# Excalibur-SLE/spmv

Hardware: AMD Instinct MI355X
Metric: fp64 CG iters/sec (SpMV effective GB/s vs HBM roofline) (higher is better)
Workload: dtype f64

## Files before the change

spmv_amd/csrc/hip/common.h:

```cpp
#pragma once

#include <mutex>
#include <vector>

#include <hip/hip_runtime.h>

#include <cstdint>
#include <cstdlib>

#include "spmv_hip.h"

struct spmv_hip_ctx {
  int device = 0;
  int num_cus = 0;
  hipStream_t stream = nullptr;
  int dot_blocks = 0;
  int64_t blas1_nt_min_elems = (int64_t)1 << 24;
  int64_t lx_min_nnz = (int64_t)1 << 20;
  int64_t lx_max_x_bytes = INT64_MAX;
  int lx_dma = 1;
  int lx_codes = 1;
  int lx_narrow_values = 1;
  int release_csr = 0;
  int64_t xw_min_nnz = (int64_t)1 << 20;
  int64_t xw_min_x_bytes = (int64_t)128 << 20;
  int xw_probe = 1;
  int csr_in_place = 0;
  int64_t lat_min_nnz = (int64_t)1 << 20;
  int bake_general = 1;
  int wdia_half = 1;
  int const_diagonals = 1;
  int const_tile = 4;
  int64_t sj_min_nnz = (int64_t)1 << 20;
  int sj_max_chunks = 432;
  int sj_wpb = 0;
  int sj_unit = 0;
  int sj_sigma = 1;
  int sym_sj_long_permille = 50;
  int sym_sj_long_rows = 1;
  int put_timeout_ms = 60000;
  std::vector<const int32_t*> watched;
  std::mutex watched_mutex;
  int poisson_skew_ppm = 0;
  int poisson_stencil = 7;
};
// ... 105 lines not shown
```

spmv_amd/csrc/hip/csr_plan.h:

```cpp
#pragma once

#include "common.h"

#include <chrono>
#include <cstdio>

constexpr int kRows = kBlock;

typedef double f64x2 __attribute__((ext_vector_type(2)));
typedef float f32x4 __attribute__((ext_vector_type(4)));
typedef int i32x2 __attribute__((ext_vector_type(2)));
typedef int i32x4 __attribute__((ext_vector_type(4)));

template <typename T>
struct VecOf;
template <>
struct VecOf<double> {
  static constexpr int V = 2;
  using val_t = f64x2;
  using col_t = i32x2;
};
template <>
struct VecOf<float> {
  static constexpr int V = 4;
// ... 288 lines not shown
  bool structure_baked() const
  {
    return row_list || lx_lidx || lat_tab || slat_mask || t_ptr || lxw_rec
           || xw_rec || wdia_val || sj_lenperm;
  }
  uint16_t* lx_lidx = nullptr;
  int32_t* lx_tab = nullptr;
  int lx = 0;
  int lx_chunks = 2;
  int lx_staged = 0;
  int lx_blocks = 0;
  int32_t* lxw_rec = nullptr;
  int lxw = 0;
  int lxw_max_cnt = 0;
  int lxw_max_pieces = 0;
  int lxw_blocks_per_cu = 0;
  uint8_t* lx_code = nullptr;
  int lx4 = 0;
  int lx4_blocks = 0;
  int lx4_lut = 1;
  float* lx_val32 = nullptr;
  const void* lx32_values0 = nullptr;
  int lx_v32 = 0;
  int32_t* xw_rec = nullptr;
  int xw = 0;
  int xw_staged = 0;
  int xw_max_cnt = 0, xw_max_pieces = 0;
  struct XwProbe* xw_probe = nullptr;
  int32_t* lat_tab = nullptr;
  uint8_t* lat_mask = nullptr;
  int lat = 0;
  int lat_blocks = 0;
  int lat_blocks_per_cu = 4;
  int lat_xcd_group = 0;
  int lat_chain = 1;

  int lattice_d1 = 0, lattice_d2 = 0;

  int32_t* zw_table = nullptr;
  int zw_slots = 0;
  int zw_grid = 0;
  int zw_segments = 0;
  int64_t zw_d2 = 0;
  int zwalk = 0;

  RowBlockOrder row_block_order(int nrb) const
// ... 71 lines not shown
                      const double* diagonal, double alpha, const double* in,
                      double beta, double* out, DotOut dot);
int spmv_slat_run_f32(const spmv_hip_csr_plan* pl, hipStream_t st,
                      const int32_t* rowptr, const float* values,
                      const float* diagonal, float alpha, const float* in,
                      float beta, float* out);
void spmv_sdia_free(spmv_hip_csr_plan* pl);
int spmv_sdia_tile_build(spmv_hip_csr_plan* pl, int R, int segments, bool force);
int spmv_sdia_bake_f64(spmv_hip_csr_plan* pl, const double* values,
                       const double* diagonal, hipStream_t st);
int spmv_sdia_bake_f32(spmv_hip_csr_plan* pl, const float* values,
                       const float* diagonal, hipStream_t st);
int spmv_sdia_grid(const spmv_hip_csr_plan* pl);
int spmv_sdia_bake_f32f64(spmv_hip_csr_plan* pl, const float* values32,
                          hipStream_t st);
int spmv_sdia_run_f32f64(const spmv_hip_csr_plan* pl, hipStream_t st,
                         double alpha, const double* in, double beta,
                         double* out, DotOut dot);
int spmv_sdia_run_f64(const spmv_hip_csr_plan* pl, hipStream_t st, double alpha,
                      const double* in, double beta, double* out, DotOut dot);
int spmv_sdia_run_f32(const spmv_hip_csr_plan* pl, hipStream_t st, float alpha,
                      const float* in, float beta, float* out);
int spmv_lxw_grid(const spmv_hip_csr_plan* pl, int elem_bytes);
int spmv_lxw_run_f64(const spmv_hip_csr_plan* pl, hipStream_t st,
                     const int32_t* rowptr, const int32_t* colind,
                     const double* values, double alpha, const double* in,
                     double beta, double* out, DotOut dot);
int spmv_lxw_run_f32f64(const spmv_hip_csr_plan* pl, hipStream_t st,
                        const int32_t* rowptr, const int32_t* colind,
                        const float* values, double alpha, const double* in,
                        double beta, double* out, DotOut dot);
int spmv_xw_grid(const spmv_hip_csr_plan* pl, int elem_bytes);
int spmv_xw_run_f64(const spmv_hip_csr_plan* pl, hipStream_t st,
                    const int32_t* rowptr, const int32_t* colind,
                    const double* values, double alpha, const double* in,
                    double beta, double* out, DotOut dot);
int spmv_xw_run_f32(const spmv_hip_csr_plan* pl, hipStream_t st,
                    const int32_t* rowptr, const int32_t* colind,
                    const float* values, float alpha, const float* in,
                    float beta, float* out);
int spmv_lxw_run_f32(const spmv_hip_csr_plan* pl, hipStream_t st,
                     const int32_t* rowptr, const int32_t* colind,
                     const float* values, float alpha, const float* in,
                     float beta, float* out);
void spmv_wdia_free(spmv_hip_csr_plan* pl);
int spmv_wdia_walk_build(spmv_hip_csr_plan* pl, int segments, bool force);
// ... 56 lines not shown
```

spmv_amd/csrc/hip/runtime.hip:

```cpp
#include "common.h"

#include <cstdio>
#include <cstring>
#include <new>

bool spmv_ctx_watch(spmv_hip_ctx* ctx, const int32_t* word, bool add)
{
  std::lock_guard<std::mutex> lock(ctx->watched_mutex);
  auto& ws = ctx->watched;
  if (add) {
    try {
      ws.push_back(word);
    } catch (...) {
      return false;
    }
    return true;
  }
  for (size_t i = 0; i < ws.size(); ++i)
    if (ws[i] == word) {
      ws[i] = ws.back();
      ws.pop_back();
      break;
    }
  return true;
// ... 121 lines not shown
}

int spmv_hip_ctx_get_option(const spmv_hip_ctx* ctx, const char* key, int64_t* value)
{
  SPMV_REQUIRE(ctx && key && value);
  if (!strcmp(key, "release_csr"))
    *value = ctx->release_csr;
  else if (!strcmp(key, "put_timeout_ms"))
    *value = ctx->put_timeout_ms;
  else if (!strcmp(key, "xw_min_nnz"))
    *value = ctx->xw_min_nnz;
  else if (!strcmp(key, "xw_min_x_bytes"))
    *value = ctx->xw_min_x_bytes;
  else if (!strcmp(key, "xw_probe"))
    *value = ctx->xw_probe;
  else if (!strcmp(key, "csr_in_place"))
    *value = ctx->csr_in_place;
  else if (!strcmp(key, "lx_min_nnz"))
    *value = ctx->lx_min_nnz;
  else if (!strcmp(key, "lat_min_nnz"))
    *value = ctx->lat_min_nnz;
  else if (!strcmp(key, "lx_narrow_values"))
    *value = ctx->lx_narrow_values;
  else if (!strcmp(key, "sj_min_nnz"))
    *value = ctx->sj_min_nnz;
  else
    return SPMV_HIP_EINVAL;
  return SPMV_HIP_OK;
}

int spmv_hip_ctx_set_option(spmv_hip_ctx* ctx, const char* key, int64_t value)
{
  SPMV_REQUIRE(ctx && key);
  if (!strcmp(key, "blas1_nt_min_elems")) {
    SPMV_REQUIRE(value >= 0);
    ctx->blas1_nt_min_elems = value;
    return SPMV_HIP_OK;
  }
  if (!strcmp(key, "lx_max_x_bytes")) {
    SPMV_REQUIRE(value >= 0);
    ctx->lx_max_x_bytes = value;
    return SPMV_HIP_OK;
  }
  if (!strcmp(key, "lx_min_nnz")) {
    SPMV_REQUIRE(value >= 0);
    ctx->lx_min_nnz = value;
// ... 27 lines not shown
  if (!strcmp(key, "lat_min_nnz")) {
    SPMV_REQUIRE(value >= 0);
    ctx->lat_min_nnz = value;
    return SPMV_HIP_OK;
  }
  if (!strcmp(key, "poisson_skew_ppm")) {
    SPMV_REQUIRE(value >= 0 && value < 1000000);
    ctx->poisson_skew_ppm = (int)value;
    return SPMV_HIP_OK;
  }
  if (!strcmp(key, "lx_dma")) {
    SPMV_REQUIRE(value == 0 || value == 1);
    ctx->lx_dma = (int)value;
    return SPMV_HIP_OK;
  }
  if (!strcmp(key, "lx_codes")) {
    SPMV_REQUIRE(value == 0 || value == 1);
    ctx->lx_codes = (int)value;
    return SPMV_HIP_OK;
  }
  if (!strcmp(key, "lx_narrow_values")) {
    SPMV_REQUIRE(value == 0 || value == 1);
    ctx->lx_narrow_values = (int)value;
    return SPMV_HIP_OK;
  }
  if (!strcmp(key, "poisson_stencil")) {
    SPMV_REQUIRE(value == 7 || value == 27);
    ctx->poisson_stencil = (int)value;
    return SPMV_HIP_OK;
  }
  if (!strcmp(key, "const_diagonals")) {
    SPMV_REQUIRE(value == 0 || value == 1);
    ctx->const_diagonals = (int)value;
    return SPMV_HIP_OK;
  }
  if (!strcmp(key, "const_tile")) {
    SPMV_REQUIRE(value == 1 || value == 2 || value == 4);
    ctx->const_tile = (int)value;
    return SPMV_HIP_OK;
  }
  if (!strcmp(key, "wdia_half")) {
    SPMV_REQUIRE(value == 0 || value == 1);
    ctx->wdia_half = (int)value;
    return SPMV_HIP_OK;
  }
  if (!strcmp(key, "sj_min_nnz")) {
// ... 264 lines not shown
```

spmv_amd/csrc/hip/spmv_csr_plan.hip:

```cpp
#include "csr_plan.h"

#include <hipcub/hipcub.hpp>

#include <algorithm>
#include <chrono>
#include <cstring>
#include <new>
#include <utility>
#include <vector>

#include "plan_malloc.h"

thread_local int64_t spmv_plan_mem_ns = 0;

namespace
{
struct MemClock {
  spmv_hip_csr_plan* pl;
  int64_t t0;
  explicit MemClock(spmv_hip_csr_plan* p = nullptr) : pl(p), t0(spmv_plan_mem_ns) {}
  ~MemClock()
  {
    if (pl)
      pl->plan_mem_us += (int)((spmv_plan_mem_ns - t0) / 1000);
// ... 65 lines not shown
}

extern "C" {

int spmv_hip_csr_plan_create(spmv_hip_ctx* ctx, int32_t num_rows,
                             int32_t num_cols, int64_t num_non_zeros,
                             const int32_t* rowptr, const int32_t* colind,
                             int symmetric, int algo, spmv_hip_csr_plan** plan)
{
  SPMV_REQUIRE(ctx && plan && num_rows >= 0 && num_cols >= 0
               && num_non_zeros >= 0);
  SPMV_REQUIRE(num_non_zeros == 0 || (rowptr && colind));
  if (num_non_zeros > 0) {
    SPMV_SET_DEVICE(ctx);
    SPMV_CHECK_HIP(hipStreamSynchronize(spmv_stream(ctx, nullptr)));
  }
  const auto t_begin = std::chrono::steady_clock::now();
  if (num_non_zeros > INT32_MAX)
    return SPMV_HIP_ERANGE;
  spmv_hip_csr_plan* pl = new (std::nothrow) spmv_hip_csr_plan;
  if (!pl)
    return SPMV_HIP_ENOMEM;
  pl->ctx = ctx;
  MemClock mem_clock(pl);
  pl->num_rows = num_rows;
  pl->num_cols = num_cols;
  pl->nnz = num_non_zeros;
  pl->symmetric = symmetric != 0;
  pl->rowptr0 = rowptr;
  pl->colind0 = colind;
  const double avg = num_rows > 0 ? (double)num_non_zeros / num_rows : 0.0;
  if (algo == SPMV_HIP_ALGO_AUTO) {
    if (!symmetric && num_non_zeros > 0 && num_non_zeros * 4 < num_rows)
      algo = SPMV_HIP_ALGO_ROWLIST;
    else
      algo = (avg <= 64.0 || num_non_zeros >= ctx->sj_min_nnz)
                 ? SPMV_HIP_ALGO_ROWBLOCK
                 : SPMV_HIP_ALGO_VECTOR;
  }
  if (algo < SPMV_HIP_ALGO_ROWBLOCK || algo > SPMV_HIP_ALGO_ROWLIST
      || (algo == SPMV_HIP_ALGO_ROWLIST && (symmetric || num_non_zeros == 0))) {
    mem_clock.pl = nullptr;
    delete pl;
    return SPMV_HIP_EINVAL;
  }
  pl->algo = algo;
// ... 366 lines not shown
    SPMV_REQUIRE(value >= 1 && value <= kBlocksPerCU);
    plan->blocks_per_cu = value;
    if (plan->zw_table && !plan->lat_tab && !plan->symmetric
        && !plan->sdia_val)
      return spmv_zwalk_order_build(plan, plan->zw_d2, spmv_walk_grid(plan), 0,
                                    true);
  } else if (!strcmp(key, "lx")) {
    SPMV_REQUIRE(value == 0 || plan->lx_lidx);
    plan->lx = value != 0;
  } else if (!strcmp(key, "lxw")) {
    SPMV_REQUIRE(value == 0 || plan->lxw_rec);
    plan->lxw = value != 0;
    if (plan->zw_table && plan->lx_lidx && !plan->lat_tab)
      return spmv_zwalk_order_build(plan, plan->zw_d2, spmv_walk_grid(plan), 0,
                                    true);
  } else if (!strcmp(key, "lx4")) {
    SPMV_REQUIRE(value == 0 || value == 1);
    SPMV_REQUIRE(value == 0 || plan->lx_code);
    plan->lx4 = value;
  } else if (!strcmp(key, "lx_v32")) {
    SPMV_REQUIRE(value == 0 || value == 1);
    SPMV_REQUIRE(value == 0 || plan->lx_val32);
    plan->lx_v32 = value;
  } else if (!strcmp(key, "lx4_lut")) {
    SPMV_REQUIRE(value == 1 || value == 2);
    plan->lx4_lut = value;
  } else if (!strcmp(key, "xw")) {
    SPMV_REQUIRE(value == 0 || plan->xw_rec);
    plan->xw = value != 0;
    if (plan->xw_probe && value) {
      plan->xw_probe->decided = 1;
      plan->xw_probe->use_xw = 1;
    }
    if (plan->zw_table && plan->xw_rec && !plan->lat_tab && !plan->lx_lidx)
      return spmv_zwalk_order_build(plan, plan->zw_d2, spmv_walk_grid(plan), 0,
                                    true);
  } else if (!strcmp(key, "xw_probe")) {
    SPMV_REQUIRE((value == 0 || value == 1) && plan->xw_rec);
    if (!plan->xw_probe)
      plan->xw_probe = new (std::nothrow) XwProbe;
    SPMV_REQUIRE(plan->xw_probe);
    xw_probe_drop_events(plan->xw_probe);
    *plan->xw_probe = XwProbe();
    plan->xw_probe->decided = value ? 0 : 1;
  } else if (!strcmp(key, "lxw_blocks_per_cu")) {
    SPMV_REQUIRE(value >= 0 && value <= kBlocksPerCU);
// ... 353 lines not shown
    *value = plan->lattice_d1;
  else if (!strcmp(key, "lattice_d2"))
    *value = plan->lattice_d2;
  else if (!strcmp(key, "lat"))
    *value = plan->lat;
  else if (!strcmp(key, "lat_chain"))
    *value = plan->lat_chain;
  else if (!strcmp(key, "lat_blocks"))
    *value = plan->lat_blocks;
  else if (!strcmp(key, "lx"))
    *value = plan->lx;
  else if (!strcmp(key, "lxw"))
    *value = plan->lxw && plan->lxw_rec ? 1 : 0;
  else if (!strcmp(key, "lx4"))
    *value = plan->lx4 && plan->lx_code ? 1 : 0;
  else if (!strcmp(key, "lx4_blocks"))
    *value = plan->lx_code ? plan->lx4_blocks : 0;
  else if (!strcmp(key, "lx4_all"))
    *value = plan->lx_code && plan->lx4_blocks == plan->lx_staged ? 1 : 0;
  else if (!strcmp(key, "lx4_lut"))
    *value = plan->lx4_lut;
  else if (!strcmp(key, "lx_v32"))
    *value = plan->lx_v32 && plan->lx_val32 ? 1 : 0;
  else if (!strcmp(key, "lxw_grid"))
    *value = plan->lxw_rec ? spmv_lxw_grid(plan, 8) : 0;
  else if (!strcmp(key, "lx_staged"))
    *value = plan->lx_staged;
  else if (!strcmp(key, "lx_blocks"))
    *value = plan->lx_blocks;
  else if (!strcmp(key, "blocks_per_cu"))
    *value = plan->blocks_per_cu;
  else if (!strcmp(key, "nontemporal"))
    *value = plan->nontemporal;
  else
    return spmv_tr_get(plan, key, value);
  return SPMV_HIP_OK;
}

}
```

spmv_amd/csrc/hip/spmv_lxw.hip:

```cpp
#include "csr_plan.h"
#include "lat_dma.h"

#include <new>
#include <type_traits>

namespace
{

struct LxwBlock {
  int rb;
  int nwin;
  int32_t a;
  int32_t cnt;
  int np;
  int own;
  int coded;
};

template <int REC>
__device__ __forceinline__ int32_t lxw_fetch(int rb,
                                             const int32_t* __restrict__ rec)
{
  int32_t w = 0;
  if (rb >= 0) {
// ... 25 lines not shown
  T y0;
};

template <typename T>
__device__ __forceinline__ LxwRegs<T> lxw_loads(const LxwBlock& blk, int t,
                                                int32_t num_rows,
                                                const int32_t* __restrict__ rowptr,
                                                const T* __restrict__ in, T beta,
                                                const T* __restrict__ out)
{
  LxwRegs<T> g;
  g.lo = g.hi = 0;
  g.y0 = T(0);
  if (blk.rb >= 0) {
    const int32_t r = blk.rb * kRows + t;
    if (r < num_rows) {
      g.lo = rowptr[r];
      g.hi = rowptr[r + 1];
      if (beta != T(0))
        g.y0 = out[r];
    }
  }
  return g;
}

template <typename TV, typename T, bool DOT, bool NT, bool TAB, bool XW, int C4>
__global__ __launch_bounds__(kBlock) void csr_lxw_kernel(
    int32_t num_rows, int32_t num_cols, int64_t nnz,
    const int32_t* __restrict__ rowptr, const int32_t* __restrict__ colind,
    const TV* __restrict__ values, const uint16_t* __restrict__ lidx,
    const uint8_t* __restrict__ code, const int32_t* __restrict__ rec, T alpha, const T* __restrict__ in, T beta,
    T* __restrict__ out, DotOut dot, RowBlockOrder ord, int vcap, int lcap,
    int xcap)
{
  using IDX = typename std::conditional<XW, int32_t, uint16_t>::type;
  constexpr int REC = XW ? kXwRec : kLxwRec;
  constexpr int IA = 16 / (int)sizeof(IDX) - 1;
  constexpr int V = 16 / (int)sizeof(TV);
  constexpr int E = 16 / (int)sizeof(T);
  constexpr int PL = kLxwPiece / E;
  extern __shared__ __attribute__((aligned(16))) unsigned char smem[];
  TV* const s_val = reinterpret_cast<TV*>(smem);
  IDX* const s_lidx
      = reinterpret_cast<IDX*>(smem + 2 * (size_t)vcap * sizeof(TV));
  T* const s_x = reinterpret_cast<T*>(smem + 2 * (size_t)vcap * sizeof(TV)
                                      + 2 * (size_t)lcap * sizeof(IDX));
// ... 74 lines not shown

  auto slot_raw = [&](int i) { return order_slot_raw_t<TAB>(ord, i, num_slots); };
  int it = blockIdx.x;
  LxwBlock cur;
  int nxt_rb;
  int32_t nxt_w;
  int32_t cur_w0;
  {
    const int rb0 = order_slot_decode(ord, slot_raw(it));
    nxt_rb = order_slot_decode(ord, slot_raw(it + stride));
    const int32_t w0 = lxw_fetch<REC>(rb0, rec);
    nxt_w = lxw_fetch<REC>(nxt_rb, rec);
    cur = lxw_decode(rb0, w0);
    cur_w0 = w0;
    issue(cur, pieces_of(w0), w0, 0);
  }
  int nn_raw = slot_raw(it + 2 * stride);
  LxwRegs<T> gA = lxw_loads<T>(cur, t, num_rows, rowptr, in, beta, out);
  LxwRegs<T> gB;
  int slot = 0;
  T y_late = T(0);
  int32_t r_late = -1;

  struct Windows {
    int32_t f[kXwMaxWin];
    int32_t d[kXwMaxWin];
  };
  auto windows_of = [&](int32_t w) {
    Windows ws;
#pragma unroll
    for (int k = 0; k < kXwMaxWin; ++k) {
      ws.f[k] = 0;
      ws.d[k] = 0;
      if constexpr (XW) {
        if (k > 0)
          ws.f[k] = __builtin_amdgcn_readlane(w, kXwFirst0 + k - 1);
        ws.d[k] = __builtin_amdgcn_readlane(w, kXwDelta0 + k);
      }
    }
    return ws;
  };
  Windows cur_ws = windows_of(cur_w0);
  struct Dict {
    int32_t w[kLxwDictSize / 2];
  };
  auto dict_of = [&](int32_t w) {
    Dict dc;
#pragma unroll
    for (int k = 0; k < kLxwDictSize / 2; ++k) {
      dc.w[k] = 0;
      if constexpr (C4 == 2)
        dc.w[k] = __builtin_amdgcn_readlane(w, kLxwDict0 + k);
    }
    return dc;
  };
  Dict cur_dc = dict_of(cur_w0);

  auto step = [&](const LxwRegs<T>& g, LxwRegs<T>& gn) {
    __builtin_amdgcn_s_waitcnt(0x0F70);
    __syncthreads();
    if (r_late >= 0)
      out[r_late] = y_late;
    r_late = -1;
    const LxwBlock nxt = lxw_decode(nxt_rb, nxt_w);
    const Windows nxt_ws = windows_of(nxt_w);
    const Dict nxt_dc = dict_of(nxt_w);
    issue(nxt, pieces_of(nxt_w), nxt_w, slot ^ 1);
    gn = lxw_loads<T>(nxt, t, num_rows, rowptr, in, beta, out);
    const int nn_rb = order_slot_decode(ord, nn_raw);
    const int32_t nn_w = lxw_fetch<REC>(nn_rb, rec);
    const int nnn_raw = slot_raw(it + 3 * stride);

    const int32_t r = cur.rb * kRows + t;
    if (cur.rb >= 0 && r < num_rows) {
      T sum = 0;
      T x_own = T(0);
      bool own_staged = false;
      int32_t j = g.lo;
      const int32_t hi = g.hi;
      if (cur.cnt > 0 && fits(cur)) {
        const TV* sv = s_val + (size_t)slot * vcap + (cur.a & (V - 1)) - cur.a;
        if (cur.nwin >= 0) {
          const IDX* sl = s_lidx + (size_t)slot * lcap + (cur.a & IA) - cur.a;
          const T* sx = s_x + (size_t)slot * xcap;
          if constexpr (DOT) {
            if (cur.own >= 0) {
              x_own = sx[cur.own + t];
              own_staged = true;
            }
          }
          if (coded(cur)) {
            const uint32_t* sc = reinterpret_cast<const uint32_t*>(
                s_lidx + (size_t)slot * lcap);
            const int32_t n0 = cur.a & ~31;
            for (; j < hi; j += 8) {
              const unsigned n = (unsigned)(j - n0);
              const uint32_t c_lo = sc[n >> 3], c_hi = sc[(n >> 3) + 1];
              const uint32_t bits
                  = __builtin_amdgcn_alignbit(c_hi, c_lo, (n & 7) * 4);
              unsigned l[8];
              T v[8], xv[8];
#pragma unroll
              for (int k = 0; k < 8; ++k) {
                const int32_t jj = j + k < hi ? j + k : hi - 1;
                v[k] = (T)sv[jj];
              }
#pragma unroll
              for (int k = 0; k < 8; ++k) {
                const unsigned c = (bits >> (4 * k)) & 15u;
                int32_t d;
                if constexpr (C4 == 1) {
                  d = reinterpret_cast<const int16_t*>(
                      s_dict + slot * (kLxwDictSize / 2))[c];
                } else {
                  const int32_t p0 = c & 2 ? cur_dc.w[1] : cur_dc.w[0];
                  const int32_t p1 = c & 2 ? cur_dc.w[3] : cur_dc.w[2];
                  const int32_t p2 = c & 2 ? cur_dc.w[5] : cur_dc.w[4];
                  const int32_t p3 = c & 2 ? cur_dc.w[7] : cur_dc.w[6];
                  const int32_t q0 = c & 4 ? p1 : p0;
                  const int32_t q1 = c & 4 ? p3 : p2;
                  const int32_t pr = c & 8 ? q1 : q0;
                  d = (int32_t)((uint32_t)pr << (16 - 16 * (int)(c & 1))) >> 16;
                }
                l[k] = j + k < hi ? (unsigned)(t + d) : 0u;
              }
#pragma unroll
              for (int k = 0; k < 8; ++k)
                xv[k] = sx[l[k]];
#pragma unroll
              for (int k = 0; k < 8; ++k)
                if (j + k < hi)
                  sum += v[k] * xv[k];
            }
          }
          for (; j < hi; j += 8) {
            unsigned l[8];
            T v[8], xv[8];
#pragma unroll
            for (int k = 0; k < 8; ++k) {
              const int32_t jj = j + k < hi ? j + k : hi - 1;
              l[k] = sl[jj];
              v[k] = (T)sv[jj];
            }
            if constexpr (XW) {
#pragma unroll
              for (int k = 0; k < 8; ++k) {
                const int32_t c = (int32_t)l[k];
                int32_t d = cur_ws.d[0];
#pragma unroll
                for (int q = 1; q < kXwMaxWin; ++q)
                  d = c >= cur_ws.f[q] ? cur_ws.d[q] : d;
                l[k] = (unsigned)(c + d);
              }
            }
#pragma unroll
            for (int k = 0; k < 8; ++k)
              xv[k] = sx[l[k]];
#pragma unroll
            for (int k = 0; k < 8; ++k)
              if (j + k < hi)
                sum += v[k] * xv[k];
          }
        } else {
          for (; j < hi; ++j)
            sum += (T)sv[j] * in[colind[j]];
        }
      } else {
        for (; j < hi; ++j)
          sum += (T)values[j] * in[colind[j]];
      }
      const T c = alpha * sum;
      T y = c;
      if (beta != T(0))
        y = c + beta * g.y0;
      y_late = y;
      r_late = r;
      if constexpr (DOT) {
        if (!own_staged)
          x_own = in[r];
        dot_acc += (double)x_own * (double)c;
      }
    }
    slot ^= 1;
    cur = nxt;
    cur_ws = nxt_ws;
    cur_dc = nxt_dc;
    nxt_rb = nn_rb;
    nxt_w = nn_w;
    nn_raw = nnn_raw;
    it += stride;
  };
  while (it < num_slots) {
    step(gA, gB);
    if (it >= num_slots)
      break;
    step(gB, gA);
  }
  if (r_late >= 0)
    out[r_late] = y_late;
  if constexpr (DOT)
    spmv_dot_epilogue(dot, dot_acc, s_red);
}

struct LxwGeom {
  int vcap, lcap, xcap;
  size_t lds;
  int per_cu;
};

LxwGeom lxw_geom(const spmv_hip_csr_plan* pl, int elem_bytes, int idx_bytes)
{
  LxwGeom g;
  const bool xw = idx_bytes == 4;
  const int V = 16 / elem_bytes;
  const int max_cnt = xw ? pl->xw_max_cnt : pl->lxw_max_cnt;
  int64_t vb = ((int64_t)(max_cnt + V) * elem_bytes + 1023) & ~1023ll;
  vb = vb < 1024 ? 1024 : (vb > 32768 ? 32768 : vb);
  g.vcap = (int)(vb / elem_bytes);
  int64_t lb = ((int64_t)(g.vcap + 8) * idx_bytes + 1023) & ~1023ll;
// ... 6 lines not shown
  per = per < 1 ? 1 : (per > kBlocksPerCU ? kBlocksPerCU : per);
  if (pl->lxw_blocks_per_cu > 0 && pl->lxw_blocks_per_cu < per)
    per = pl->lxw_blocks_per_cu;
  g.per_cu = per;
  return g;
}

int lxw_grid(const spmv_hip_csr_plan* pl, int elem_bytes, int idx_bytes)
{
  const LxwGeom g = lxw_geom(pl, elem_bytes, idx_bytes);
  const int nrb = (pl->num_rows + kRows - 1) / kRows;
  int grid = pl->ctx->num_cus * g.per_cu;
  if (grid > pl->ctx->dot_blocks)
    grid = pl->ctx->dot_blocks;
  if (grid > nrb)
    grid = nrb;
  if (grid < 1)
    grid = 1;
  if (grid >= 8)
    grid -= grid % 8;
  return grid;
}

template <typename TV, typename T, bool DOT, bool XW, int C4>
int lxw_launch_c(const spmv_hip_csr_plan* pl, hipStream_t st,
                 const int32_t* rowptr, const int32_t* colind, const TV* values,
                 T alpha, const T* in, T beta, T* out, DotOut dot)
{
  const LxwGeom g = lxw_geom(pl, (int)sizeof(T), XW ? 4 : 2);
  const int vcap = g.vcap * (int)(sizeof(T) / sizeof(TV));
  const int nrb = (pl->num_rows + kRows - 1) / kRows;
  const int grid = lxw_grid(pl, (int)sizeof(T), XW ? 4 : 2);
  RowBlockOrder ord = pl->row_block_order(nrb);
  ord.xcd_group = pl->lat_xcd_group;
  if (pl->zwalk && pl->zw_table && pl->zw_grid == grid) {
    ord.table = pl->zw_table;
    ord.num_slots = pl->zw_slots;
  }
  auto kern
      = ord.table
            ? (pl->nontemporal ? csr_lxw_kernel<TV, T, DOT, true, true, XW, C4>
                               : csr_lxw_kernel<TV, T, DOT, false, true, XW, C4>)
            : (pl->nontemporal ? csr_lxw_kernel<TV, T, DOT, true, false, XW, C4>
                               : csr_lxw_kernel<TV, T, DOT, false, false, XW, C4>);
  if (g.lds > 48 * 1024)
    SPMV_CHECK_HIP(hipFuncSetAttribute(
        reinterpret_cast<const void*>(kern),
        hipFuncAttributeMaxDynamicSharedMemorySize, (int)g.lds));
  hipLaunchKernelGGL(kern, dim3(grid), dim3(kBlock), g.lds, st, pl->num_rows,
                     pl->num_cols, pl->nnz, rowptr, colind, values,
                     XW ? nullptr : pl->lx_lidx, C4 ? pl->lx_code : nullptr,
// ... 7 lines not shown
int lxw_launch(const spmv_hip_csr_plan* pl, hipStream_t st,
               const int32_t* rowptr, const int32_t* colind, const TV* values,
               T alpha, const T* in, T beta, T* out, DotOut dot)
{
  if constexpr (!XW) {
    if (pl->lx4 && pl->lx_code)
      return pl->lx4_lut == 2
                 ? lxw_launch_c<TV, T, DOT, XW, 2>(pl, st, rowptr, colind, values,
                                                   alpha, in, beta, out, dot)
                 : lxw_launch_c<TV, T, DOT, XW, 1>(pl, st, rowptr, colind, values,
                                                   alpha, in, beta, out, dot);
  }
  return lxw_launch_c<TV, T, DOT, XW, 0>(pl, st, rowptr, colind, values, alpha,
                                         in, beta, out, dot);
}

}

int spmv_lxw_grid(const spmv_hip_csr_plan* pl, int elem_bytes)
{
  return lxw_grid(pl, elem_bytes, 2);
}

int spmv_xw_grid(const spmv_hip_csr_plan* pl, int elem_bytes)
{
  return lxw_grid(pl, elem_bytes, 4);
}

int spmv_lxw_run_f64(const spmv_hip_csr_plan* pl, hipStream_t st,
                     const int32_t* rowptr, const int32_t* colind,
                     const double* values, double alpha, const double* in,
                     double beta, double* out, DotOut dot)
{
  if (dot.partials)
    return lxw_launch<double, double, true, false>(pl, st, rowptr, colind, values,
                                                   alpha, in, beta, out, dot);
  return lxw_launch<double, double, false, false>(pl, st, rowptr, colind, values,
                                                  alpha, in, beta, out, dot);
}

int spmv_lxw_run_f32f64(const spmv_hip_csr_plan* pl, hipStream_t st,
                        const int32_t* rowptr, const int32_t* colind,
                        const float* values, double alpha, const double* in,
                        double beta, double* out, DotOut dot)
{
  if (dot.partials)
// ... 36 lines not shown
```

Measured before the change: 298.4.

## Add three-deep LDS ring kernel with dedicated producer waves for LXW SpMV

Adds a new f64 LXW SpMV kernel in which two extra producer wavefronts per block DMA values, index codes, rowptr, y and staged x pieces into a three-slot LDS ring, while the four compute waves consume earlier slots. Row pointers and the beta*y input now come from LDS, and the row-sum loop is factored into a shared helper. The goal is deeper prefetch and overlap of memory traffic with compute than the previous double-buffered loop gave. In exchange it uses more LDS per block, which can lower occupancy, and adds barrier coordination between producer and consumer waves. The ring is on by default when the geometry fits, with a knob to fall back to depth 2.

```diff
diff --git a/spmv_amd/csrc/hip/common.h b/spmv_amd/csrc/hip/common.h
--- a/spmv_amd/csrc/hip/common.h
+++ b/spmv_amd/csrc/hip/common.h
@@ -10,6 +10,10 @@
 
 #include "spmv_hip.h"
 
+#ifndef SPMV_LX_RING_DEFAULT
+#define SPMV_LX_RING_DEFAULT 3
+#endif
+
 struct spmv_hip_ctx {
   int device = 0;
   int num_cus = 0;
@@ -21,6 +25,7 @@
   int lx_dma = 1;
   int lx_codes = 1;
   int lx_narrow_values = 1;
+  int lx_ring = SPMV_LX_RING_DEFAULT;
   int release_csr = 0;
   int64_t xw_min_nnz = (int64_t)1 << 20;
   int64_t xw_min_x_bytes = (int64_t)128 << 20;
diff --git a/spmv_amd/csrc/hip/csr_plan.h b/spmv_amd/csrc/hip/csr_plan.h
--- a/spmv_amd/csrc/hip/csr_plan.h
+++ b/spmv_amd/csrc/hip/csr_plan.h
@@ -334,6 +334,7 @@
   float* lx_val32 = nullptr;
   const void* lx32_values0 = nullptr;
   int lx_v32 = 0;
+  int lx_ring = SPMV_LX_RING_DEFAULT;
   int32_t* xw_rec = nullptr;
   int xw = 0;
   int xw_staged = 0;
@@ -451,6 +452,7 @@
 int spmv_sdia_run_f32(const spmv_hip_csr_plan* pl, hipStream_t st, float alpha,
                       const float* in, float beta, float* out);
 int spmv_lxw_grid(const spmv_hip_csr_plan* pl, int elem_bytes);
+int spmv_lxw_ring(const spmv_hip_csr_plan* pl, int* lds_bytes);
 int spmv_lxw_run_f64(const spmv_hip_csr_plan* pl, hipStream_t st,
                      const int32_t* rowptr, const int32_t* colind,
                      const double* values, double alpha, const double* in,
diff --git a/spmv_amd/csrc/hip/runtime.hip b/spmv_amd/csrc/hip/runtime.hip
--- a/spmv_amd/csrc/hip/runtime.hip
+++ b/spmv_amd/csrc/hip/runtime.hip
@@ -167,6 +167,8 @@
     *value = ctx->lat_min_nnz;
   else if (!strcmp(key, "lx_narrow_values"))
     *value = ctx->lx_narrow_values;
+  else if (!strcmp(key, "lx_ring"))
+    *value = ctx->lx_ring;
   else if (!strcmp(key, "sj_min_nnz"))
     *value = ctx->sj_min_nnz;
   else
@@ -240,6 +242,11 @@
   if (!strcmp(key, "lx_narrow_values")) {
     SPMV_REQUIRE(value == 0 || value == 1);
     ctx->lx_narrow_values = (int)value;
+    return SPMV_HIP_OK;
+  }
+  if (!strcmp(key, "lx_ring")) {
+    SPMV_REQUIRE(value == 2 || value == 3);
+    ctx->lx_ring = (int)value;
     return SPMV_HIP_OK;
   }
   if (!strcmp(key, "poisson_stencil")) {
diff --git a/spmv_amd/csrc/hip/spmv_csr_plan.hip b/spmv_amd/csrc/hip/spmv_csr_plan.hip
--- a/spmv_amd/csrc/hip/spmv_csr_plan.hip
+++ b/spmv_amd/csrc/hip/spmv_csr_plan.hip
@@ -111,6 +111,7 @@
   if (!pl)
     return SPMV_HIP_ENOMEM;
   pl->ctx = ctx;
+  pl->lx_ring = ctx->lx_ring;
   MemClock mem_clock(pl);
   pl->num_rows = num_rows;
   pl->num_cols = num_cols;
@@ -523,6 +524,14 @@
     SPMV_REQUIRE(value == 0 || value == 1);
     SPMV_REQUIRE(value == 0 || plan->lx_val32);
     plan->lx_v32 = value;
+  } else if (!strcmp(key, "lx_ring")) {
+    SPMV_REQUIRE(value == 2 || value == 3);
+    const int before = plan->lx_ring;
+    plan->lx_ring = value;
+    if (value == 3 && spmv_lxw_ring(plan, nullptr) != 3) {
+      plan->lx_ring = before;
+      return SPMV_HIP_EINVAL;
+    }
   } else if (!strcmp(key, "lx4_lut")) {
     SPMV_REQUIRE(value == 1 || value == 2);
     plan->lx4_lut = value;
@@ -922,6 +931,10 @@
     *value = plan->lx4_lut;
   else if (!strcmp(key, "lx_v32"))
     *value = plan->lx_v32 && plan->lx_val32 ? 1 : 0;
+  else if (!strcmp(key, "lx_ring"))
+    *value = spmv_lxw_ring(plan, nullptr);
+  else if (!strcmp(key, "lx_ring_lds"))
+    (void)spmv_lxw_ring(plan, value);
   else if (!strcmp(key, "lxw_grid"))
     *value = plan->lxw_rec ? spmv_lxw_grid(plan, 8) : 0;
   else if (!strcmp(key, "lx_staged"))
diff --git a/spmv_amd/csrc/hip/spmv_lxw.hip b/spmv_amd/csrc/hip/spmv_lxw.hip
--- a/spmv_amd/csrc/hip/spmv_lxw.hip
+++ b/spmv_amd/csrc/hip/spmv_lxw.hip
@@ -71,6 +71,122 @@
     }
   }
   return g;
+}
+
+struct LxwWindows {
+  int32_t f[kXwMaxWin];
+  int32_t d[kXwMaxWin];
+};
+struct LxwDict {
+  int32_t w[kLxwDictSize / 2];
+};
+template <bool ON>
+__device__ __forceinline__ LxwDict lxw_dict_of(int32_t w)
+{
+  LxwDict dc;
+#pragma unroll
+  for (int k = 0; k < kLxwDictSize / 2; ++k) {
+    dc.w[k] = 0;
+    if constexpr (ON)
+      dc.w[k] = __builtin_amdgcn_readlane(w, kLxwDict0 + k);
+  }
+  return dc;
+}
+
+template <typename TV, typename T, typename IDX, bool XW, int C4>
+__device__ __forceinline__ T lxw_row_sum(
+    int t, int32_t j, const int32_t hi, const LxwBlock& cur, bool fit,
+    bool is_coded, const TV* sv_slot, const IDX* sl_slot, const T* sx,
+    const int32_t* dict, const LxwWindows& cur_ws, const LxwDict& cur_dc,
+    const TV* __restrict__ values, const int32_t* __restrict__ colind,
+    const T* __restrict__ in)
+{
+  constexpr int IA = 16 / (int)sizeof(IDX) - 1;
+  constexpr int V = 16 / (int)sizeof(TV);
+  T sum = 0;
+  if (fit) {
+    const TV* sv = sv_slot + (cur.a & (V - 1)) - cur.a;
+    if (cur.nwin >= 0) {
+      const IDX* sl = sl_slot + (cur.a & IA) - cur.a;
+      if (is_coded) {
+        const uint32_t* sc = reinterpret_cast<const uint32_t*>(sl_slot);
+        const int32_t n0 = cur.a & ~31;
+        for (; j < hi; j += 8) {
+          const unsigned n = (unsigned)(j - n0);
+          const uint32_t c_lo = sc[n >> 3], c_hi = sc[(n >> 3) + 1];
+          const uint32_t bits
+              = __builtin_amdgcn_alignbit(c_hi, c_lo, (n & 7) * 4);
+          unsigned l[8];
+          T v[8], xv[8];
+#pragma unroll
+          for (int k = 0; k < 8; ++k) {
+            const int32_t jj = j + k < hi ? j + k : hi - 1;
+            v[k] = (T)sv[jj];
+          }
+#pragma unroll
+          for (int k = 0; k < 8; ++k) {
+            const unsigned c = (bits >> (4 * k)) & 15u;
+            int32_t d;
+            if constexpr (C4 == 1) {
+              d = reinterpret_cast<const int16_t*>(dict)[c];
+            } else {
+              const int32_t p0 = c & 2 ? cur_dc.w[1] : cur_dc.w[0];
+              const int32_t p1 = c & 2 ? cur_dc.w[3] : cur_dc.w[2];
+              const int32_t p2 = c & 2 ? cur_dc.w[5] : cur_dc.w[4];
+              const int32_t p3 = c & 2 ? cur_dc.w[7] : cur_dc.w[6];
+              const int32_t q0 = c & 4 ? p1 : p0;
+              const int32_t q1 = c & 4 ? p3 : p2;
+              const int32_t pr = c & 8 ? q1 : q0;
+              d = (int32_t)((uint32_t)pr << (16 - 16 * (int)(c & 1))) >> 16;
+            }
+            l[k] = j + k < hi ? (unsigned)(t + d) : 0u;
+          }
+#pragma unroll
+          for (int k = 0; k < 8; ++k)
+            xv[k] = sx[l[k]];
+#pragma unroll
+          for (int k = 0; k < 8; ++k)
+            if (j + k < hi)
+              sum += v[k] * xv[k];
+        }
+      }
+      for (; j < hi; j += 8) {
+        unsigned l[8];
+        T v[8], xv[8];
+#pragma unroll
+        for (int k = 0; k < 8; ++k) {
+          const int32_t jj = j + k < hi ? j + k : hi - 1;
+          l[k] = sl[jj];
+          v[k] = (T)sv[jj];
+        }
+        if constexpr (XW) {
+#pragma unroll
+          for (int k = 0; k < 8; ++k) {
+            const int32_t c = (int32_t)l[k];
+            int32_t d = cur_ws.d[0];
+#pragma unroll
+            for (int q = 1; q < kXwMaxWin; ++q)
+              d = c >= cur_ws.f[q] ? cur_ws.d[q] : d;
+            l[k] = (unsigned)(c + d);
+          }
+        }
+#pragma unroll
+        for (int k = 0; k < 8; ++k)
+          xv[k] = sx[l[k]];
+#pragma unroll
+        for (int k = 0; k < 8; ++k)
+          if (j + k < hi)
+            sum += v[k] * xv[k];
+      }
+    } else {
+      for (; j < hi; ++j)
+        sum += (T)sv[j] * in[colind[j]];
+    }
+  } else {
+    for (; j < hi; ++j)
+      sum += (T)values[j] * in[colind[j]];
+  }
+  return sum;
 }
 
 template <typename TV, typename T, bool DOT, bool NT, bool TAB, bool XW, int C4>
@@ -191,10 +307,7 @@
   T y_late = T(0);
   int32_t r_late = -1;
 
-  struct Windows {
-    int32_t f[kXwMaxWin];
-    int32_t d[kXwMaxWin];
-  };
+  using Windows = LxwWindows;
   auto windows_of = [&](int32_t w) {
     Windows ws;
 #pragma unroll
@@ -210,19 +323,8 @@
     return ws;
   };
   Windows cur_ws = windows_of(cur_w0);
-  struct Dict {
-    int32_t w[kLxwDictSize / 2];
-  };
-  auto dict_of = [&](int32_t w) {
-    Dict dc;
-#pragma unroll
-    for (int k = 0; k < kLxwDictSize / 2; ++k) {
-      dc.w[k] = 0;
-      if constexpr (C4 == 2)
-        dc.w[k] = __builtin_amdgcn_readlane(w, kLxwDict0 + k);
-    }
-    return dc;
-  };
+  using Dict = LxwDict;
+  auto dict_of = [&](int32_t w) { return lxw_dict_of<C4 == 2>(w); };
   Dict cur_dc = dict_of(cur_w0);
 
   auto step = [&](const LxwRegs<T>& g, LxwRegs<T>& gn) {
@@ -242,102 +344,20 @@
 
     const int32_t r = cur.rb * kRows + t;
     if (cur.rb >= 0 && r < num_rows) {
-      T sum = 0;
       T x_own = T(0);
       bool own_staged = false;
-      int32_t j = g.lo;
-      const int32_t hi = g.hi;
-      if (cur.cnt > 0 && fits(cur)) {
-        const TV* sv = s_val + (size_t)slot * vcap + (cur.a & (V - 1)) - cur.a;
-        if (cur.nwin >= 0) {
-          const IDX* sl = s_lidx + (size_t)slot * lcap + (cur.a & IA) - cur.a;
-          const T* sx = s_x + (size_t)slot * xcap;
-          if constexpr (DOT) {
-            if (cur.own >= 0) {
-              x_own = sx[cur.own + t];
-              own_staged = true;
-            }
-          }
-          if (coded(cur)) {
-            const uint32_t* sc = reinterpret_cast<const uint32_t*>(
-                s_lidx + (size_t)slot * lcap);
-            const int32_t n0 = cur.a & ~31;
-            for (; j < hi; j += 8) {
-              const unsigned n = (unsigned)(j - n0);
-              const uint32_t c_lo = sc[n >> 3], c_hi = sc[(n >> 3) + 1];
-              const uint32_t bits
-                  = __builtin_amdgcn_alignbit(c_hi, c_lo, (n & 7) * 4);
-              unsigned l[8];
-              T v[8], xv[8];
-#pragma unroll
-              for (int k = 0; k < 8; ++k) {
-                const int32_t jj = j + k < hi ? j + k : hi - 1;
-                v[k] = (T)sv[jj];
-              }
-#pragma unroll
-              for (int k = 0; k < 8; ++k) {
-                const unsigned c = (bits >> (4 * k)) & 15u;
-                int32_t d;
-                if constexpr (C4 == 1) {
-                  d = reinterpret_cast<const int16_t*>(
-                      s_dict + slot * (kLxwDictSize / 2))[c];
-                } else {
-                  const int32_t p0 = c & 2 ? cur_dc.w[1] : cur_dc.w[0];
-                  const int32_t p1 = c & 2 ? cur_dc.w[3] : cur_dc.w[2];
-                  const int32_t p2 = c & 2 ? cur_dc.w[5] : cur_dc.w[4];
-                  const int32_t p3 = c & 2 ? cur_dc.w[7] : cur_dc.w[6];
-                  const int32_t q0 = c & 4 ? p1 : p0;
-                  const int32_t q1 = c & 4 ? p3 : p2;
-                  const int32_t pr = c & 8 ? q1 : q0;
-                  d = (int32_t)((uint32_t)pr << (16 - 16 * (int)(c & 1))) >> 16;
-                }
-                l[k] = j + k < hi ? (unsigned)(t + d) : 0u;
-              }
-#pragma unroll
-              for (int k = 0; k < 8; ++k)
-                xv[k] = sx[l[k]];
-#pragma unroll
-              for (int k = 0; k < 8; ++k)
-                if (j + k < hi)
-                  sum += v[k] * xv[k];
-            }
-          }
-          for (; j < hi; j += 8) {
-            unsigned l[8];
-            T v[8], xv[8];
-#pragma unroll
-            for (int k = 0; k < 8; ++k) {
-              const int32_t jj = j + k < hi ? j + k : hi - 1;
-              l[k] = sl[jj];
-              v[k] = (T)sv[jj];
-            }
-            if constexpr (XW) {
-#pragma unroll
-              for (int k = 0; k < 8; ++k) {
-                const int32_t c = (int32_t)l[k];
-                int32_t d = cur_ws.d[0];
-#pragma unroll
-                for (int q = 1; q < kXwMaxWin; ++q)
-                  d = c >= cur_ws.f[q] ? cur_ws.d[q] : d;
-                l[k] = (unsigned)(c + d);
-              }
-            }
-#pragma unroll
-            for (int k = 0; k < 8; ++k)
-              xv[k] = sx[l[k]];
-#pragma unroll
-            for (int k = 0; k < 8; ++k)
-              if (j + k < hi)
-                sum += v[k] * xv[k];
-          }
-        } else {
-          for (; j < hi; ++j)
-            sum += (T)sv[j] * in[colind[j]];
+      const bool fit = cur.cnt > 0 && fits(cur);
+      const T* const sx = s_x + (size_t)slot * xcap;
+      if constexpr (DOT) {
+        if (fit && cur.nwin >= 0 && cur.own >= 0) {
+          x_own = sx[cur.own + t];
+          own_staged = true;
         }
-      } else {
-        for (; j < hi; ++j)
-          sum += (T)values[j] * in[colind[j]];
-      }
+      }
+      const T sum = lxw_row_sum<TV, T, IDX, XW, C4>(
+          t, g.lo, g.hi, cur, fit, coded(cur), s_val + (size_t)slot * vcap,
+          s_lidx + (size_t)slot * lcap, sx, s_dict + slot * (kLxwDictSize / 2),
+          cur_ws, cur_dc, values, colind, in);
       const T c = alpha * sum;
       T y = c;
       if (beta != T(0))
@@ -364,6 +384,225 @@
     if (it >= num_slots)
       break;
     step(gB, gA);
+  }
+  if (r_late >= 0)
+    out[r_late] = y_late;
+  if constexpr (DOT)
+    spmv_dot_epilogue(dot, dot_acc, s_red);
+}
+
+constexpr int kRingDepth = 3;
+constexpr int kRingProducers = 2;
+constexpr int kRingBlock = kBlock + 64 * kRingProducers;
+constexpr int kRingRpBytes = (kRows + 1 + 3) / 4 * 16;
+constexpr int kRingHdrWords = 32;
+constexpr int kRingHdrBytes = kRingHdrWords * 4;
+static_assert(kLxwRec < kRingHdrWords, "the header holds a record and the row block");
+
+template <typename TT, bool NT>
+__device__ __forceinline__ void ring_dma(const TT* __restrict__ p, int64_t len,
+                                         int64_t base, int64_t b, TT* s_slot,
+                                         int cap, int lane)
+{
+  constexpr int V = 16 / (int)sizeof(TT);
+  if (b <= base)
+    return;
+  const int64_t jclamp = (b - 1) & ~(int64_t)(V - 1);
+  if (jclamp + V <= len) {
+    const unsigned lds0 = (unsigned)(uintptr_t)(
+        (__attribute__((address_space(3))) void*)s_slot);
+    const int pieces = (int)(((b - base) * (int64_t)sizeof(TT) + 1023) >> 10);
+    for (int q = 0; q < pieces; ++q) {
+      const int c = q * 64 + lane;
+      const int64_t j = base + (int64_t)c * V;
+      if (j <= jclamp && c * 16 + 16 <= cap)
+        glds16<NT>(p + j, lds0 + (unsigned)q * 1024u);
+    }
+  } else {
+    for (int64_t j = base + lane; j < b; j += 64)
+      if ((j - base + 1) * (int64_t)sizeof(TT) <= cap)
+        s_slot[j - base] = p[j];
+  }
+}
+
+template <typename TV, typename T, bool DOT, bool NT, bool TAB, int C4>
+__global__ __launch_bounds__(kRingBlock) void csr_lxw_ring_kernel(
+    int32_t num_rows, int32_t num_cols, int64_t nnz,
+    const int32_t* __restrict__ rowptr, const int32_t* __restrict__ colind,
+    const TV* __restrict__ values, const uint16_t* __restrict__ lidx,
+    const uint8_t* __restrict__ code, const int32_t* __restrict__ rec, T alpha,
+    const T* __restrict__ in, T beta, T* out, DotOut dot, RowBlockOrder ord,
+    int vcap, int ibytes, int xcap)
+{
+  constexpr int V = 16 / (int)sizeof(TV);
+  constexpr int E = 16 / (int)sizeof(T);
+  constexpr int PL = kLxwPiece / E;
+  extern __shared__ __attribute__((aligned(16))) unsigned char smem[];
+  const int vbytes = vcap * (int)sizeof(TV);
+  const int xbytes = xcap * (int)sizeof(T);
+  const int o_idx = vbytes, o_x = o_idx + ibytes, o_rp = o_x + xbytes,
+            o_y = o_rp + kRingRpBytes, o_hdr = o_y + kRows * (int)sizeof(T);
+  const int slot_bytes = o_hdr + kRingHdrBytes;
+  __shared__ double s_red[kRingBlock / 64];
+
+  const int t = threadIdx.x;
+  const int wave = __builtin_amdgcn_readfirstlane(t >> 6);
+  const int lane = t & 63;
+  const int stride = gridDim.x;
+  const int num_slots = order_slots(ord);
+  const int32_t col_last = (num_cols - E) & ~(E - 1);
+
+  auto coded = [&](const LxwBlock& b) {
+    if constexpr (C4 != 0)
+      return b.coded != 0 && (b.cnt + (b.a & 31) + 7) / 8 * 4 + 8 <= ibytes;
+    else
+      return false;
+  };
+  auto fits = [&](const LxwBlock& b) {
+    return b.cnt + (b.a & (V - 1)) <= vcap
+           && (b.nwin < 0 || coded(b)
+               || (b.cnt + (b.a & 7)) * 2 <= ibytes);
+  };
+
+  if (wave >= kBlock / 64) {
+    const int par = wave - kBlock / 64;
+    const int64_t code_len = lx_code_bytes(nnz);
+    const int64_t val_len = std::is_same<TV, T>::value ? nnz : lx32_len(nnz);
+    auto slot_raw
+        = [&](int i) { return order_slot_raw_t<TAB>(ord, i, num_slots); };
+    auto issue = [&](int rb, int32_t w, int sl) {
+      unsigned char* const s0 = smem + (size_t)sl * slot_bytes;
+      if (lane < kRingHdrWords)
+        reinterpret_cast<int32_t*>(s0 + o_hdr)[lane]
+            = lane == kRingHdrWords - 1 ? rb : w;
+      if (rb < 0)
+        return;
+      const LxwBlock b = lxw_decode(rb, w);
+      int32_t pc[kLxwMaxPieces];
+#pragma unroll
+      for (int p = 0; p < kLxwMaxPieces; ++p)
+        pc[p] = __builtin_amdgcn_readlane(w, kLxwPieces0 + p);
+      const int64_t r0 = (int64_t)rb * kRows;
+      const int64_t r1 = r0 + kRows < num_rows ? r0 + kRows : num_rows;
+      ring_dma<int32_t, false>(rowptr, (int64_t)num_rows + 1, r0, r1 + 1,
+                               reinterpret_cast<int32_t*>(s0 + o_rp),
+                               kRingRpBytes, lane);
+      if (beta != T(0))
+        ring_dma<T, false>(out, num_rows, r0, r1,
+                           reinterpret_cast<T*>(s0 + o_y),
+                           kRows * (int)sizeof(T), lane);
+      if (b.cnt <= 0 || !fits(b))
+        return;
+      const int64_t a = b.a, e = (int64_t)b.a + b.cnt;
+      ring_dma<TV, NT>(values, val_len, a & ~(int64_t)(V - 1), e,
+                       reinterpret_cast<TV*>(s0), vbytes, lane);
+      if (b.nwin < 0)
+        return;
+      if (coded(b))
+        ring_dma<uint8_t, NT>(code, code_len, (a >> 1) & ~(int64_t)15,
+                              (e + 1) >> 1, s0 + o_idx, ibytes, lane);
+      else
+        ring_dma<uint16_t, NT>(lidx, nnz + 8, a & ~(int64_t)7, e,
+                               reinterpret_cast<uint16_t*>(s0 + o_idx), ibytes,
+                               lane);
+      const unsigned ldsx = (unsigned)(uintptr_t)(
+          (__attribute__((address_space(3))) void*)(s0 + o_x));
+#pragma unroll
+      for (int p = 0; p < kLxwMaxPieces; ++p) {
+        if (p >= b.np || (p + 1) * kLxwPiece > xcap)
+          continue;
+        if (lane < PL) {
+          int32_t c = pc[p] + lane * E;
+          c = c < col_last ? c : col_last;
+          glds16<false>(in + c,
+                        ldsx + (unsigned)(p * kLxwPiece * (int)sizeof(T)));
+        }
+      }
+    };
+    int pit = blockIdx.x + par * stride;
+    int sl = par;
+    const int rb0 = order_slot_decode(ord, slot_raw(pit));
+    int nxt_rb = order_slot_decode(ord, slot_raw(pit + 2 * stride));
+    int nn_raw = slot_raw(pit + 4 * stride);
+    const int32_t w0 = lxw_fetch<kLxwRec>(rb0, rec);
+    int32_t nxt_w = lxw_fetch<kLxwRec>(nxt_rb, rec);
+    issue(rb0, w0, sl);
+    pit += 2 * stride;
+    sl = (sl + 2) % kRingDepth;
+    int s = 0;
+    for (int it = blockIdx.x; it < num_slots; it += stride, ++s) {
+      if ((s & 1) == par) {
+        __builtin_amdgcn_s_waitcnt(0x0070);
+        __atomic_signal_fence(__ATOMIC_SEQ_CST);
+        __builtin_amdgcn_s_barrier();
+        __atomic_signal_fence(__ATOMIC_SEQ_CST);
+        const int nn_rb = order_slot_decode(ord, nn_raw);
+        issue(nxt_rb, nxt_w, sl);
+        pit += 2 * stride;
+        sl = (sl + 2) % kRingDepth;
+        nxt_rb = nn_rb;
+        nxt_w = lxw_fetch<kLxwRec>(nxt_rb, rec);
+        nn_raw = slot_raw(pit + 2 * stride);
+      } else {
+        __builtin_amdgcn_s_waitcnt(0xC07F);
+        __atomic_signal_fence(__ATOMIC_SEQ_CST);
+        __builtin_amdgcn_s_barrier();
+        __atomic_signal_fence(__ATOMIC_SEQ_CST);
+      }
+    }
+    if constexpr (DOT)
+      spmv_dot_epilogue(dot, 0.0, s_red);
+    return;
+  }
+
+  double dot_acc = 0.0;
+  T y_late = T(0);
+  int32_t r_late = -1;
+  int slot = 0;
+  const LxwWindows no_ws{};
+  for (int it = blockIdx.x; it < num_slots; it += stride) {
+    __builtin_amdgcn_s_waitcnt(0x0F70);
+    __syncthreads();
+    if (r_late >= 0)
+      out[r_late] = y_late;
+    r_late = -1;
+    const unsigned char* const s0 = smem + (size_t)slot * slot_bytes;
+    const int32_t* const hdr = reinterpret_cast<const int32_t*>(s0 + o_hdr);
+    const int32_t cur_w = hdr[lane < kRingHdrWords ? lane : kRingHdrWords - 1];
+    const LxwBlock cur = lxw_decode(
+        __builtin_amdgcn_readlane(cur_w, kRingHdrWords - 1), cur_w);
+    LxwDict cur_dc = lxw_dict_of<C4 == 2>(cur_w);
+    const int32_t r = cur.rb * kRows + t;
+    if (cur.rb >= 0 && r < num_rows) {
+      const int32_t* const rp = reinterpret_cast<const int32_t*>(s0 + o_rp);
+      const T* const sx = reinterpret_cast<const T*>(s0 + o_x);
+      const bool fit = cur.cnt > 0 && fits(cur);
+      T x_own = T(0);
+      bool own_staged = false;
+      if constexpr (DOT) {
+        if (fit && cur.nwin >= 0 && cur.own >= 0) {
+          x_own = sx[cur.own + t];
+          own_staged = true;
+        }
+      }
+      const T sum = lxw_row_sum<TV, T, uint16_t, false, C4>(
+          t, rp[t], rp[t + 1], cur, fit, coded(cur),
+          reinterpret_cast<const TV*>(s0),
+          reinterpret_cast<const uint16_t*>(s0 + o_idx), sx,
+          hdr + kLxwDict0, no_ws, cur_dc, values, colind, in);
+      const T c = alpha * sum;
+      T y = c;
+      if (beta != T(0))
+        y = c + beta * reinterpret_cast<const T*>(s0 + o_y)[t];
+      y_late = y;
+      r_late = r;
+      if constexpr (DOT) {
+        if (!own_staged)
+          x_own = in[r];
+        dot_acc += (double)x_own * (double)c;
+      }
+    }
+    slot = slot + 1 == kRingDepth ? 0 : slot + 1;
   }
   if (r_late >= 0)
     out[r_late] = y_late;
@@ -416,11 +655,80 @@
   return grid;
 }
 
+struct LxwRing {
+  int vcap, ibytes, xcap;
+  size_t lds;
+  bool ok;
+};
+
+LxwRing lxw_ring_geom(const spmv_hip_csr_plan* pl, int val_bytes, int elem_bytes)
+{
+  LxwRing r{};
+  const int V = 16 / val_bytes;
+  const int64_t vb = ((int64_t)(pl->lxw_max_cnt + V) * val_bytes + 15) & ~15ll;
+  const bool codes_only = pl->lx4 && pl->lx_code && pl->lx4_blocks == pl->lx_staged;
+  const int64_t ib = codes_only ? (pl->lxw_max_cnt / 2 + 48 + 15) & ~15ll
+                                : ((int64_t)(pl->lxw_max_cnt + 16) * 2 + 15) & ~15ll;
+  const int np = pl->lxw_max_pieces < 1 ? 1 : pl->lxw_max_pieces;
+  const int64_t slot = vb + ib + (int64_t)np * kLxwPiece * elem_bytes + kRingRpBytes
+                       + kRows * elem_bytes + kRingHdrBytes;
+  const int64_t lds = kRingDepth * slot;
+  const LxwGeom g = lxw_geom(pl, elem_bytes, 2);
+  r.ok = elem_bytes == 8 && pl->lxw_rec && np <= kLxwMaxPieces
+         && lds + 64 <= 160 * 1024 - 1024
+         && (160 * 1024 - 1024) / (lds + 64) >= g.per_cu;
+  r.vcap = (int)(vb / val_bytes);
+  r.ibytes = (int)ib;
+  r.xcap = np * kLxwPiece;
+  r.lds = (size_t)lds;
+  return r;
+}
+
+template <typename TV, typename T, bool DOT, int C4>
+int lxw_ring_launch(const spmv_hip_csr_plan* pl, hipStream_t st, const LxwRing& r,
+                    const int32_t* rowptr, const int32_t* colind, const TV* values,
+                    T alpha, const T* in, T beta, T* out, DotOut dot)
+{
+  const int nrb = (pl->num_rows + kRows - 1) / kRows;
+  const int grid = lxw_grid(pl, (int)sizeof(T), 2);
+  RowBlockOrder ord = pl->row_block_order(nrb);
+  ord.xcd_group = pl->lat_xcd_group;
+  if (pl->zwalk && pl->zw_table && pl->zw_grid == grid) {
+    ord.table = pl->zw_table;
+    ord.num_slots = pl->zw_slots;
+  }
+  auto kern
+      = ord.table
+            ? (pl->nontemporal ? csr_lxw_ring_kernel<TV, T, DOT, true, true, C4>
+                               : csr_lxw_ring_kernel<TV, T, DOT, false, true, C4>)
+            : (pl->nontemporal ? csr_lxw_ring_kernel<TV, T, DOT, true, false, C4>
+                               : csr_lxw_ring_kernel<TV, T, DOT, false, false, C4>);
+  if (r.lds > 48 * 1024)
+    SPMV_CHECK_HIP(hipFuncSetAttribute(
+        reinterpret_cast<const void*>(kern),
+        hipFuncAttributeMaxDynamicSharedMemorySize, (int)r.lds));
+  hipLaunchKernelGGL(kern, dim3(grid), dim3(kRingBlock), r.lds, st, pl->num_rows,
+                     pl->num_cols, pl->nnz, rowptr, colind, values, pl->lx_lidx,
+                     C4 ? pl->lx_code : nullptr, pl->lxw_rec, alpha, in, beta, out,
+                     dot, ord, r.vcap, r.ibytes, r.xcap);
+  SPMV_CHECK_LAUNCH();
+  return SPMV_HIP_OK;
+}
+
 template <typename TV, typename T, bool DOT, bool XW, int C4>
 int lxw_launch_c(const spmv_hip_csr_plan* pl, hipStream_t st,
                  const int32_t* rowptr, const int32_t* colind, const TV* values,
                  T alpha, const T* in, T beta, T* out, DotOut dot)
 {
+  if constexpr (!XW && sizeof(T) == 8) {
+    if (pl->lx_ring == kRingDepth && aligned16(rowptr)
+        && (beta == T(0) || aligned16(out))) {
+      const LxwRing r = lxw_ring_geom(pl, (int)sizeof(TV), (int)sizeof(T));
+      if (r.ok)
+        return lxw_ring_launch<TV, T, DOT, C4>(pl, st, r, rowptr, colind, values,
+                                               alpha, in, beta, out, dot);
+    }
+  }
   const LxwGeom g = lxw_geom(pl, (int)sizeof(T), XW ? 4 : 2);
   const int vcap = g.vcap * (int)(sizeof(T) / sizeof(TV));
   const int nrb = (pl->num_rows + kRows - 1) / kRows;
@@ -474,6 +782,23 @@
   return lxw_grid(pl, elem_bytes, 2);
 }
 
+int spmv_lxw_ring(const spmv_hip_csr_plan* pl, int* lds_bytes)
+{
+  int depth = 2;
+  size_t lds = 0;
+  if (pl->lxw_rec) {
+    lds = lxw_geom(pl, 8, 2).lds;
+    const LxwRing r = lxw_ring_geom(pl, pl->lx_v32 && pl->lx_val32 ? 4 : 8, 8);
+    if (pl->lx_ring == kRingDepth && r.ok && aligned16(pl->rowptr0)) {
+      depth = kRingDepth;
+      lds = r.lds;
+    }
+  }
+  if (lds_bytes)
+    *lds_bytes = (int)lds;
+  return depth;
+}
+
 int spmv_xw_grid(const spmv_hip_csr_plan* pl, int elem_bytes)
 {
   return lxw_grid(pl, elem_bytes, 4);
```

After: 248.5. 0.833x the previous value.
